# ZihanLiao/pytorch-kaldi-resnet

Measured on AMD Instinct MI355X. Metric: utterances/sec (300-frame x 80 fbank, bs256/GPU), ResNet-34 + AAM-softmax training step, higher is better.
Workload: dtype f32 (operands as 2 fp16 terms of value x 2^k, 3 cross products, f32 accumulate); 1 GPU; BASELINE configs[1]: ResNet-34 + AAM-softmax (m 0.2, s 30), 1211 speakers, 300-frame x 80 fbank, per-GPU batch 256, fwd+CE+bwd+SGD(0.9, wd 5e-4); global_batch=256, frames=300, feat_dim=80, parallelism=dp1, launch=hipGraph replay (1 graph), mfma=f16x3

## Files before the change

### include/spkhip.h

```cpp
#ifndef SPKHIP_H
#define SPKHIP_H
#include <stddef.h>
#ifdef __cplusplus
extern "C" {
#endif

int spk_version(void);
const char* spk_last_error(void);
int spk_build_flags(void);

#define SPK_IN_AFFINE_RELU 1
#define SPK_EPI_AFFINE 2
#define SPK_EPI_ADD 4
#define SPK_EPI_RELU 8
#define SPK_EPI_STATS 16
#define SPK_IN_BNBWD 64
#define SPK_EPI_BNBWD 32

#define SPK_CONV_WS 128
#define SPK_CONV_PIPE 1024

#define SPK_CONV_M16 (1 << 17)

#define SPK_WGRAD_GROUPS 2048
// ... 33 lines not shown
                      unsigned* side_amax, const int* wlen , void* stream);

int spk_conv_wgrad_limits(int WN, int* max_halo_pix , int* max_tile_pix );
size_t spk_conv_wgrad_workspace(int nsplit, int ksize, int Cin, int Cout);
int spk_conv3x3_c32_stream(const float* in, const float* wpk, float* out, const float* in_scale, const float* in_shift, float* stats,
                           int B, int H, int W, int flags, const unsigned* in_amax, unsigned* out_amax, int nblocks, void* stream);
int spk_conv1x1_stream(const float* in, const float* wpk, float* out, const float* in_scale, const float* in_shift,
                       const float* epi_add, const unsigned* add_mask, const float* bn_raw, const unsigned* bn_mask,
                       const float* bn4, float* stats, long long P, int C, int flags, const unsigned* in_amax, unsigned* out_amax,
                       int nblocks, void* stream);
int spk_conv1x1_stream_rows(int nblocks, int C);
int spk_wgrad_reduce(const float* partial, float* dw, int nslab, int ksize, int Cin, int Cout, int accumulate, void* stream);
int spk_conv_wgrad(const float* x, const float* dy, float* dw, float* partial, const float* in_scale,
                   const float* in_shift, int B, int IH, int IW, int Cin, int OH, int OW, int Cout, int ksize, int stride,
                   int TH, int TW, int WN, int nsplit, int flags, int accumulate, int split , const unsigned* dy_amax , const unsigned* x_amax , void* stream);

int spk_stem_fwd_blocks(int B, int F, int T);
int spk_stem_conv_fwd(const float* x, const float* w, float* out, float* stats, const float* epi_scale,
                      const float* epi_shift, int B, int F, int T, int flags,
                      unsigned* amax_out , void* stream);
int spk_stem_conv_fwd_len(const float* x, const float* w, float* out, float* stats, const float* epi_scale,
                          const float* epi_shift, int B, int F, int T, int flags, unsigned* amax_out, const int* len ,
                          void* stream);
int spk_stem_wgrad_blocks(int B, int F, int T);
int spk_stem_conv_wgrad(const float* x, const float* draw, float* dw, float* partial, int B, int F, int T,
                        int accumulate, void* stream);
int spk_stem_stats(const float* x, const float* w, float* stats, int B, int F, int T, void* stream);
int spk_stem_fwd_apply(const float* x, const float* w, const float* scale, const float* shift, float* raw_out, float* act_out,
                       unsigned* mask_out, unsigned* amax_out, int B, int F, int T, void* stream);
int spk_stem_bwd_wgrad(const float* x, const float* d, const float* raw, const float* mean, const float* invstd,
// ... 156 lines not shown
```

### pytorch-kaldi-resnet_amd/csrc/conv_kernel.h

```cpp
#pragma once
#include "spk_common.h"
#include <type_traits>

#ifndef STAGE_U
#define STAGE_U 4
#endif
#ifndef CONV_NT
#define CONV_NT 3
#endif
static __device__ __forceinline__ void conv_st(float* p, f32x4 v) {
    if constexpr ((CONV_NT & 1) != 0) __builtin_nontemporal_store(v, (f32x4*)p);
    else *(f32x4*)p = v;
}
template <int BIT>
static __device__ __forceinline__ f32x4 conv_ld(const float* p) {
    if constexpr ((CONV_NT & BIT) != 0) return __builtin_nontemporal_load((const f32x4*)p);
    else return *(const f32x4*)p;
}
#ifndef STAGE_U2
#define STAGE_U2 2
#endif
#ifndef STAGE_U2_C32
#define STAGE_U2_C32 4
#endif
// ... 42 lines not shown
    int halo_h, halo_w, min_dy, min_dx;
    unsigned halo_w_magic;
    int ntaps, ncg, nblocks, flags;
    int tap_off[18];
    int tap_w[18];
    int tap_g[18];
    const unsigned* in_amax;
    float in_sigma;
    const unsigned* w_amax;
    unsigned* out_amax;
    unsigned* side_amax;
    const int* wlen;
    int tap_boff[9];
    int kc;
};

#define PIPE_D 3
#ifndef PIPE16_D
#define PIPE16_D 3
#endif
#ifndef PIPE16_D_CONV
#define PIPE16_D_CONV 3
#endif
#ifndef PIPE_VPM
#define PIPE_VPM 6
#endif
#ifdef CONV_STAMPS
#define CONV_STAMP_BLOCKS 4096
static __device__ unsigned long long g_conv_stamps[CONV_STAMP_BLOCKS][16];
#define STAMP(i) do { if (threadIdx.x == 0 && blockIdx.x < CONV_STAMP_BLOCKS) g_conv_stamps[blockIdx.x][i] = __builtin_amdgcn_s_memtime(); } while (0)
// ... 1121 lines not shown
```

### pytorch-kaldi-resnet_amd/csrc/conv_mfma.hip

```cpp
#include "conv_kernel.h"

int spk_launch_conv_split(const ConvArgs& a, size_t lds_bytes, int MT, int NT, int split, int ck, hipStream_t st);
int spk_launch_conv_pipe(const ConvArgs& a, size_t lds_bytes, int MT, int NT, hipStream_t st);
int spk_launch_conv_ws(const ConvArgs& a, int MT, int NT, int WC, int split, int lp4, hipStream_t st);

template <int MT, int NT>
static int launch_conv(const ConvArgs& a, size_t lds_bytes, hipStream_t st) {
    if (a.flags & SPK_IN_BNBWD)
        hipLaunchKernelGGL((conv_mfma_kernel<MT, NT, true, 0>), dim3(a.nblocks), dim3(256), lds_bytes, st, a);
    else if (a.flags & SPK_EPI_WMASK)
        hipLaunchKernelGGL((conv_mfma_kernel<MT, NT, false, 0, SPK_EPI_WMASK>), dim3(a.nblocks), dim3(256), lds_bytes, st, a);
    else
        hipLaunchKernelGGL((conv_mfma_kernel<MT, NT, false, 0>), dim3(a.nblocks), dim3(256), lds_bytes, st, a);
    SPK_LAUNCH_CHECK("spk_conv_mfma");
    return 0;
}

static int conv_mfma_entry(const float* in, const float* wpk, float* out, const float* in_scale,
                             const float* in_shift, const float* epi_scale, const float* epi_shift,
                             const float* epi_add, const float* in_raw, const float* in_act, const float* in_bn4,
                             const float* in_coef, const unsigned* in_mask, const unsigned* bn_mask, const unsigned* add_mask, float* side_draw,
                             float* side_dz,
                             const float* bn_raw,
                             const float* bn_act, const float* bn4, float* stats, int B, int IH, int IW, int Cin, int OH,
// ... 137 lines not shown
            SPK_REQUIRE((Cin / SPK_SPLIT_CK) % 2 == 0, "spk_conv_mfma: CONV_M16 walks the 16-channel planes in pairs");
        }
        a.flags = flags & ~SPK_CONV_PIPE;
        return spk_launch_conv_pipe(a, lds2, MT, NT, st);
    }
    if (split) return spk_launch_conv_split(a, lds_bytes, MT, NT, split, ck, st);
#define CASE(M, N) if (MT == M && NT == N) return launch_conv<M, N>(a, lds_bytes, st)
    CASE(1, 1); CASE(2, 1); CASE(3, 1); CASE(4, 1);
    CASE(1, 2); CASE(2, 2); CASE(3, 2); CASE(4, 2);
    CASE(1, 4); CASE(2, 4);
#undef CASE
    spk_set_error("spk_conv_mfma: unsupported tile config MT=%d NT=%d", MT, NT);
    return -1;
}

extern "C" int spk_conv_mfma(const float* in, const float* wpk, float* out, const float* in_scale,
                             const float* in_shift, const float* epi_scale, const float* epi_shift,
                             const float* epi_add, const float* in_raw, const float* in_act, const float* in_bn4,
                             const float* in_coef, const unsigned* in_mask, const unsigned* bn_mask, const unsigned* add_mask, float* side_draw,
                             float* side_dz, const float* bn_raw, const float* bn_act, const float* bn4, float* stats, int B, int IH,
                             int IW, int Cin, int OH, int OW, int OHf, int OWf, int Cout, int IS, int OS, int ooy, int oox, int ntaps,
                             const int* tap_dy, const int* tap_dx, const int* tap_w, int TH, int TW, int MT,
                             int NT, int kc, int ips, int flags, int split, const unsigned* in_amax, unsigned* out_amax,
                             unsigned* side_amax, void* stream) {
    return conv_mfma_entry(in, wpk, out, in_scale, in_shift, epi_scale, epi_shift, epi_add, in_raw, in_act, in_bn4, in_coef, in_mask,
                           bn_mask, add_mask, side_draw, side_dz, bn_raw, bn_act, bn4, stats, B, IH, IW, Cin, OH, OW, OHf, OWf, Cout, IS,
                           OS, ooy, oox, ntaps, tap_dy, tap_dx, tap_w, TH, TW, MT, NT, kc, ips, flags, split, in_amax, out_amax,
                           side_amax, nullptr, stream);
}

// ... 16 lines not shown
```

### pytorch-kaldi-resnet_amd/csrc/conv_pipe.hip

```cpp
#include "conv_kernel.h"

template <int MT, int NT>
static int launch_pipe(const ConvArgs& a, size_t lds_bytes, hipStream_t st) {
    if (a.flags & SPK_IN_BNBWD) {
#ifndef SPK_EXPERIMENTAL
        spk_set_error("spk_conv_mfma: the pipelined fused-BatchNorm-backward kernel is an experimental form: build with SPK_EXPERIMENTAL=1");
        return -1;
#else
        if constexpr (MT * NT <= 4) {
            SPK_REQUIRE(a.in_mask, "spk_conv_mfma: the pipelined fused-BatchNorm-backward kernel takes the ReLU mask as sign bits");
            hipLaunchKernelGGL((conv_pipe_kernel<MT, NT, true, true>), dim3(a.nblocks), dim3(256), lds_bytes, st, a);
        } else {
            spk_set_error("spk_conv_mfma: no pipelined fused-BatchNorm-backward kernel for MT=%d NT=%d", MT, NT);
            return -1;
        }
#endif
    } else if (a.flags & SPK_CONV_M16) {
        ConvArgs b = a;
        b.flags = a.flags & ~SPK_CONV_M16;
        if constexpr (MT == 3 && NT == 2) {
            const int var = b.flags | (b.add_mask ? SPK_FL_ADDMASK : 0) | (b.bn_mask ? SPK_FL_BNMASK : 0) | (b.bn_act ? (1 << 30) : 0);
#define LP(PREV, VV) hipLaunchKernelGGL((conv_pipe_kernel<MT, NT, false, false, PREV, true, VV>), dim3(a.nblocks), dim3(256), lds_bytes, st, b)
            if (b.flags & SPK_EPI_WMASK) {
                LP(false, SPK_EPI_WMASK);
                SPK_LAUNCH_CHECK("spk_conv_mfma(pipe)");
                return 0;
            }
#ifdef SPK_NO_FL_VARIANTS
            if (a.flags & SPK_IN_PRESPLIT) LP(true, -1); else LP(false, -1);
#else
            switch (var) {
#ifdef SPK_FL_FWD_PIPE
                case SPK_IN_AFFINE_RELU | SPK_EPI_STATS: LP(false, SPK_IN_AFFINE_RELU | SPK_EPI_STATS); break;
                case SPK_EPI_STATS: LP(false, SPK_EPI_STATS); break;
#endif
                case SPK_IN_PRESPLIT | SPK_EPI_STATS | SPK_EPI_BNBWD: LP(true, SPK_IN_PRESPLIT | SPK_EPI_STATS | SPK_EPI_BNBWD); break;
                case SPK_IN_PRESPLIT | SPK_EPI_ADD | SPK_EPI_STATS | SPK_EPI_BNBWD | SPK_FL_ADDMASK | SPK_FL_BNMASK:
                    LP(true, SPK_IN_PRESPLIT | SPK_EPI_ADD | SPK_EPI_STATS | SPK_EPI_BNBWD | SPK_FL_ADDMASK | SPK_FL_BNMASK); break;
                case SPK_IN_PRESPLIT | SPK_EPI_ADD | SPK_FL_ADDMASK: LP(true, SPK_IN_PRESPLIT | SPK_EPI_ADD | SPK_FL_ADDMASK); break;
                default:
                    if (a.flags & SPK_IN_PRESPLIT) LP(true, -1); else LP(false, -1);
            }
#endif
#undef LP
        } else {
            spk_set_error("spk_conv_mfma: no 16x16x32 pipelined kernel for MT=%d NT=%d", MT, NT);
            return -1;
        }
    } else if (a.flags & SPK_EPI_WMASK)
        hipLaunchKernelGGL((conv_pipe_kernel<MT, NT, false, false, false, false, SPK_EPI_WMASK>), dim3(a.nblocks), dim3(256), lds_bytes, st, a);
    else if (a.flags & SPK_IN_PRESPLIT)
        hipLaunchKernelGGL((conv_pipe_kernel<MT, NT, false, false, true>), dim3(a.nblocks), dim3(256), lds_bytes, st, a);
    else
        hipLaunchKernelGGL((conv_pipe_kernel<MT, NT, false>), dim3(a.nblocks), dim3(256), lds_bytes, st, a);
    SPK_LAUNCH_CHECK("spk_conv_mfma(pipe)");
    return 0;
}

int spk_launch_conv_pipe(const ConvArgs& a, size_t lds_bytes, int MT, int NT, hipStream_t st) {
#define CASE(M, N) if (MT == M && NT == N) return launch_pipe<M, N>(a, lds_bytes, st);
    CASE(2, 1) CASE(3, 1) CASE(1, 2) CASE(2, 2) CASE(3, 2) CASE(1, 4)
#undef CASE
    spk_set_error("spk_conv_mfma: unsupported pipelined tile config MT=%d NT=%d", MT, NT);
    return -1;
}

#ifdef CONV_STAMPS
extern "C" int spk_debug_stamps_pipe(unsigned long long* out, int nblocks) {
    if (nblocks < 0) {
// ... 9 lines not shown
```

### pytorch-kaldi-resnet_amd/csrc/conv_split.hip

```cpp
#include "conv_kernel.h"

template <int MT, int NT>
static int launch_split_ck32(const ConvArgs& a, size_t lds_bytes, hipStream_t st) {
#ifndef SPK_NO_FL_VARIANTS
    const int var = a.flags | (a.add_mask ? SPK_FL_ADDMASK : 0) | (a.bn_mask ? SPK_FL_BNMASK : 0) | (a.in_mask ? SPK_FL_INMASK : 0);
    constexpr int V2 = SPK_IN_BNBWD | SPK_SIDE_PRESPLIT | SPK_EPI_STATS | SPK_EPI_BNBWD | SPK_FL_INMASK;
    constexpr int V1 = SPK_IN_BNBWD | SPK_SIDE_PRESPLIT | SPK_EPI_ADD | SPK_EPI_STATS | SPK_EPI_BNBWD | SPK_FL_ADDMASK | SPK_FL_BNMASK;
    if (!a.in_act && !a.bn_act && !a.side_dz && var == V2)
        hipLaunchKernelGGL((conv_mfma_kernel<MT, NT, true, 3, V2, 32>), dim3(a.nblocks), dim3(256), lds_bytes, st, a);
    else if (!a.in_act && !a.bn_act && !a.side_dz && var == V1)
        hipLaunchKernelGGL((conv_mfma_kernel<MT, NT, true, 3, V1, 32>), dim3(a.nblocks), dim3(256), lds_bytes, st, a);
    else
#endif
        hipLaunchKernelGGL((conv_mfma_kernel<MT, NT, true, 3, -1, 32>), dim3(a.nblocks), dim3(256), lds_bytes, st, a);
    SPK_LAUNCH_CHECK("spk_conv_mfma(split, 32-channel planes)");
    return 0;
}

template <int MT, int NT, int SPLIT>
static int launch_split(const ConvArgs& a, size_t lds_bytes, hipStream_t st) {
    if (a.flags & SPK_IN_BNBWD) {
#ifndef SPK_NO_FL_VARIANTS
        if constexpr (SPLIT == 3 && MT == 2 && NT == 1) {
            const int var = a.flags | (a.add_mask ? SPK_FL_ADDMASK : 0) | (a.bn_mask ? SPK_FL_BNMASK : 0) | (a.in_mask ? SPK_FL_INMASK : 0);
            constexpr int V2 = SPK_IN_BNBWD | SPK_SIDE_PRESPLIT | SPK_EPI_STATS | SPK_EPI_BNBWD | SPK_FL_INMASK;
            constexpr int V1 = SPK_IN_BNBWD | SPK_SIDE_PRESPLIT | SPK_EPI_ADD | SPK_EPI_STATS | SPK_EPI_BNBWD | SPK_FL_ADDMASK | SPK_FL_BNMASK;
            if (!a.in_act && !a.bn_act && !a.side_dz && (var == V1 || var == V2)) {
                if (var == V2) hipLaunchKernelGGL((conv_mfma_kernel<MT, NT, true, SPLIT, V2>), dim3(a.nblocks), dim3(256), lds_bytes, st, a);
                else hipLaunchKernelGGL((conv_mfma_kernel<MT, NT, true, SPLIT, V1>), dim3(a.nblocks), dim3(256), lds_bytes, st, a);
                SPK_LAUNCH_CHECK("spk_conv_mfma(split)");
                return 0;
            }
        }
#endif
        hipLaunchKernelGGL((conv_mfma_kernel<MT, NT, true, SPLIT>), dim3(a.nblocks), dim3(256), lds_bytes, st, a);
    } else if (a.flags & SPK_EPI_WMASK) {
        hipLaunchKernelGGL((conv_mfma_kernel<MT, NT, false, SPLIT, SPK_EPI_WMASK>), dim3(a.nblocks), dim3(256), lds_bytes, st, a);
    } else {
#ifndef SPK_NO_FL_VARIANTS
        if constexpr (SPLIT == 3 && ((MT == 2 && NT == 1) || (MT == 1 && NT == 2) || (MT == 2 && NT == 2))) {
            if (!a.add_mask && !a.bn_mask && !a.bn_act) {
                if (a.flags == (SPK_IN_AFFINE_RELU | SPK_EPI_STATS)) {
                    hipLaunchKernelGGL((conv_mfma_kernel<MT, NT, false, SPLIT, SPK_IN_AFFINE_RELU | SPK_EPI_STATS>), dim3(a.nblocks), dim3(256), lds_bytes, st, a);
                    SPK_LAUNCH_CHECK("spk_conv_mfma(split)");
                    return 0;
                }
                if (a.flags == SPK_EPI_STATS) {
                    hipLaunchKernelGGL((conv_mfma_kernel<MT, NT, false, SPLIT, SPK_EPI_STATS>), dim3(a.nblocks), dim3(256), lds_bytes, st, a);
                    SPK_LAUNCH_CHECK("spk_conv_mfma(split)");
                    return 0;
                }
            }
        }
#endif
        hipLaunchKernelGGL((conv_mfma_kernel<MT, NT, false, SPLIT>), dim3(a.nblocks), dim3(256), lds_bytes, st, a);
    }
    SPK_LAUNCH_CHECK("spk_conv_mfma(split)");
    return 0;
}

int spk_launch_conv_split(const ConvArgs& a, size_t lds_bytes, int MT, int NT, int split, int ck, hipStream_t st) {
    if (ck == 32) {
        if (MT == 2 && NT == 1) return launch_split_ck32<2, 1>(a, lds_bytes, st);
        if (MT == 1 && NT == 1) return launch_split_ck32<1, 1>(a, lds_bytes, st);
        spk_set_error("spk_conv_mfma: 32-channel planes are instantiated for MT=2 / MT=1 with NT=1, not MT=%d NT=%d", MT, NT);
        return -1;
    }
#define CASE(M, N)                                                      \
    if (MT == M && NT == N) {                                           \
// ... 22 lines not shown
```

### pytorch-kaldi-resnet_amd/csrc/conv_wgrad.hip

```cpp
#include "conv_wgrad.h"

int spk_launch_wgrad_split(const WgradArgs& a, int WN, int split, hipStream_t st);
int spk_launch_wgrad_ws(const WgradArgs& a, int WN, hipStream_t st);
int spk_launch_wgrad_pipe(const WgradArgs& a, int WN, hipStream_t st);
int spk_launch_wgrad_1x1(const WgradArgs& a, int WN, int CG, hipStream_t st);
int spk_launch_wgrad_wm16(const WgradArgs& a, hipStream_t st);
int spk_launch_wgrad_c32m16(const WgradArgs& a, hipStream_t st);
int spk_launch_wgrad_wm(const WgradArgs& a, hipStream_t st);

template <int NTAPS, int WK, int WN>
__global__ __launch_bounds__(256, 2) void conv_wgrad_kernel(WgradArgs a) {
    extern __shared__ __attribute__((aligned(16))) float lds[];
    const int tid = threadIdx.x, lane = tid & 63;
    const int wave = __builtin_amdgcn_readfirstlane(tid >> 6);
    const int r = lane & 31, h = lane >> 5;
    const int wk = wave / WN, wn = wave % WN;
    const int ci0 = blockIdx.y * 32;
    const int co0 = blockIdx.z * (32 * WN);
    const int halo_pix = a.halo_h * a.halo_w;
    const int npix = a.TH * a.TW;
    float* xs = lds;
    float* dys = lds + halo_pix * 32;
    const int flags = a.flags;

// ... 160 lines not shown
            }
        }
    }
    if (wk == 0) {
        float* slab = a.partial + (size_t)blockIdx.x * NTAPS * a.Cin * a.Cout;
#pragma unroll
        for (int t = 0; t < NTAPS; ++t)
#pragma unroll
            for (int e = 0; e < 16; ++e) {
                const int row = (e & 3) + 8 * (e >> 2) + 4 * h;
                slab[((size_t)t * a.Cin + ci0 + row) * a.Cout + co0 + wn * 32 + r] = acc[t][e];
            }
    }
}

__global__ void wgrad_reduce_kernel(const float* __restrict__ partial, float* __restrict__ dw, int nslab, int ntaps,
                                    int Cin, int Cout, int accumulate) {
    const int idx = blockIdx.x * blockDim.x + threadIdx.x;
    const int total = ntaps * Cin * Cout;
    if (idx >= total) return;
    float s0 = 0.f, s1 = 0.f, s2 = 0.f, s3 = 0.f;
    int k = 0;
    for (; k + 4 <= nslab; k += 4) {
        s0 += partial[(size_t)(k + 0) * total + idx];
        s1 += partial[(size_t)(k + 1) * total + idx];
        s2 += partial[(size_t)(k + 2) * total + idx];
        s3 += partial[(size_t)(k + 3) * total + idx];
    }
    for (; k < nslab; ++k) s0 += partial[(size_t)k * total + idx];
    const float s = (s0 + s1) + (s2 + s3);
    const int co = idx % Cout;
    const int ci = (idx / Cout) % Cin;
    const int t = idx / (Cout * Cin);
    float* dst = dw + ((size_t)co * Cin + ci) * ntaps + t;
    *dst = accumulate ? *dst + s : s;
}

// ... 12 lines not shown
    return 0;
}

extern "C" size_t spk_conv_wgrad_workspace(int nsplit, int ksize, int Cin, int Cout) {
    return (size_t)nsplit * ksize * ksize * Cin * Cout * sizeof(float);
}

extern "C" int spk_wgrad_reduce(const float* partial, float* dw, int nslab, int ksize, int Cin, int Cout, int accumulate,
                                void* stream) {
    SPK_REQUIRE(partial && dw && nslab >= 1 && (ksize == 1 || ksize == 3), "spk_wgrad_reduce: bad arguments");
    const int ntaps = ksize * ksize, total = ntaps * Cin * Cout;
    hipLaunchKernelGGL(wgrad_reduce_kernel, dim3(spk_ceil_div(total, 256)), dim3(256), 0, (hipStream_t)stream, partial, dw, nslab,
                       ntaps, Cin, Cout, accumulate);
    SPK_LAUNCH_CHECK("spk_wgrad_reduce");
    return 0;
}

extern "C" int spk_conv_wgrad(const float* x, const float* dy, float* dw, float* partial, const float* in_scale,
                              const float* in_shift, int B, int IH, int IW, int Cin, int OH, int OW, int Cout,
                              int ksize, int stride, int TH, int TW, int WN, int nsplit, int flags, int accumulate,
                              int split, const unsigned* dy_amax, const unsigned* x_amax, void* stream) {
    SPK_REQUIRE(x && dy && dw && partial, "spk_conv_wgrad: null pointer");
    SPK_REQUIRE(!(flags & SPK_EPI_WMASK), "spk_conv_wgrad: SPK_EPI_WMASK is a forward-epilogue flag (spk_conv_mfma_len)");
    SPK_REQUIRE(ksize == 1 || ksize == 3, "spk_conv_wgrad: ksize=%d unsupported", ksize);
    SPK_REQUIRE(Cin % 32 == 0 && Cout % 32 == 0, "spk_conv_wgrad: channels (%d,%d) must be multiples of 32", Cin, Cout);
    SPK_REQUIRE(WN == 1 || WN == 2 || WN == 4, "spk_conv_wgrad: WN=%d", WN);
    SPK_REQUIRE(Cout % (32 * WN) == 0, "spk_conv_wgrad: Cout=%d not a multiple of 32*WN", Cout);
    SPK_REQUIRE(TH >= 1 && TW >= 2 && (TW % 2) == 0, "spk_conv_wgrad: TW=%d must be even", TW);
    SPK_REQUIRE(nsplit >= 1, "spk_conv_wgrad: nsplit");
    SPK_REQUIRE(!(flags & SPK_IN_AFFINE_RELU) || (in_scale && in_shift), "spk_conv_wgrad: IN_AFFINE_RELU needs scale/shift");
// ... 80 lines not shown
```

### pytorch-kaldi-resnet_amd/csrc/conv_wgrad_split.hip

```cpp
#include "conv_wgrad.h"

typedef short s16x4 __attribute__((ext_vector_type(4)));
typedef short s16x8 __attribute__((ext_vector_type(8)));
typedef __attribute__((address_space(3))) s16x4 lds_s16x4;

static __device__ __forceinline__ s16x8 tr_read8(const unsigned char* p0, const unsigned char* p1) {
#ifdef WG_ABL_NO_FRAG
    s16x8 v = {1, 2, 3, 4, 5, 6, 7, 8};
    asm volatile("" : "+v"(v) : "v"(p0), "v"(p1));
    return v;
#endif
    const s16x4 lo = __builtin_amdgcn_ds_read_tr16_b64_v4i16((lds_s16x4*)p0);
    const s16x4 hi = __builtin_amdgcn_ds_read_tr16_b64_v4i16((lds_s16x4*)p1);
    return __builtin_shufflevector(lo, hi, 0, 1, 2, 3, 4, 5, 6, 7);
}

#ifndef WGRAD_XCD_BAND
#define WGRAD_XCD_BAND 1
#endif
struct WgradBlock { int g, ci0, co0; };
template <int WN>
static __device__ __forceinline__ WgradBlock wgrad_block(const WgradArgs& a) {
    const int ncgi = a.Cin >> 5, M = ncgi * (a.Cout / (32 * WN));
    const int bid = blockIdx.x;
// ... 493 lines not shown
    if (a.halo_h * a.halo_w <= 32 * 4) hipLaunchKernelGGL((conv_wgrad_ws_kernel<NTAPS, WK, WN, 4>), grid, dim3(512), lds_bytes, st, a);
    else hipLaunchKernelGGL((conv_wgrad_ws_kernel<NTAPS, WK, WN, WGRAD_NX>), grid, dim3(512), lds_bytes, st, a);
    SPK_LAUNCH_CHECK("spk_conv_wgrad(ws)");
    return 0;
}

int spk_launch_wgrad_ws(const WgradArgs& a, int WN, hipStream_t st) {
    SPK_REQUIRE(a.KW == 3, "spk_conv_wgrad(ws): 3x3 only");
    if (WN == 1) return launch_ws<9, 4, 1>(a, st);
    if (WN == 2) return launch_ws<9, 2, 2>(a, st);
    return launch_ws<9, 1, 4>(a, st);
}

#endif

template <int NTAPS, int WK, int WN>
static int launch_one(const WgradArgs& a, int split, hipStream_t st) {
    const int npix_pad = ((a.TH * a.TW + 15) >> 4) << 4;
    constexpr int PD = WN * 192 + (WN > 1 ? 64 : 0);
    size_t lds_bytes = (size_t)a.halo_h * a.halo_w * 192 + (size_t)npix_pad * PD;
    const size_t red_bytes = (WK > 1) ? (size_t)WN * NTAPS * 16 * 64 * sizeof(float) : 0;
    if (lds_bytes < red_bytes) lds_bytes = red_bytes;
    SPK_REQUIRE(lds_bytes <= 160 * 1024, "spk_conv_wgrad(split): tile %dx%d needs %zu B of LDS", a.TH, a.TW, lds_bytes);
    dim3 grid(a.nsplit * (a.Cin / 32) * (a.Cout / (32 * WN)));
    const bool small = a.halo_h * a.halo_w <= 32 * 4;
    if (split == 3) {
        const int var = ((a.flags & SPK_IN_AFFINE_RELU) ? 1 : 0) | ((a.flags & SPK_DY_PRESPLIT) ? 2 : 0);
        if constexpr (NTAPS == 9 && WK == 4 && WN == 1) {
            if (!small && var == 3) {
                hipLaunchKernelGGL((conv_wgrad_split_kernel<NTAPS, WK, WN, 3, WGRAD_NX, 3>), grid, dim3(256), lds_bytes, st, a);
                SPK_LAUNCH_CHECK("spk_conv_wgrad(split)");
                return 0;
            }
            if (!small && var == 2) {
                hipLaunchKernelGGL((conv_wgrad_split_kernel<NTAPS, WK, WN, 3, WGRAD_NX, 2>), grid, dim3(256), lds_bytes, st, a);
                SPK_LAUNCH_CHECK("spk_conv_wgrad(split)");
                return 0;
            }
        }
        if (small) hipLaunchKernelGGL((conv_wgrad_split_kernel<NTAPS, WK, WN, 3, 4>), grid, dim3(256), lds_bytes, st, a);
        else hipLaunchKernelGGL((conv_wgrad_split_kernel<NTAPS, WK, WN, 3, WGRAD_NX>), grid, dim3(256), lds_bytes, st, a);
    } else if constexpr (NTAPS == 9) {
        if (split == 6) {
            if (small) hipLaunchKernelGGL((conv_wgrad_split_kernel<9, WK, WN, 6, 4>), grid, dim3(256), lds_bytes, st, a);
            else hipLaunchKernelGGL((conv_wgrad_split_kernel<9, WK, WN, 6, WGRAD_NX>), grid, dim3(256), lds_bytes, st, a);
        } else {
            if (small) hipLaunchKernelGGL((conv_wgrad_split_kernel<9, WK, WN, 9, 4>), grid, dim3(256), lds_bytes, st, a);
            else hipLaunchKernelGGL((conv_wgrad_split_kernel<9, WK, WN, 9, WGRAD_NX>), grid, dim3(256), lds_bytes, st, a);
        }
    } else {
        spk_set_error("spk_conv_wgrad(split): 1x1 weight gradients exist in the f16x3 mode only");
        return -1;
    }
    SPK_LAUNCH_CHECK("spk_conv_wgrad(split)");
    return 0;
// ... 13 lines not shown
```

### pytorch-kaldi-resnet_amd/csrc/err.cpp

```cpp
#include <stdarg.h>
#include <stdio.h>
#include "spk_common.h"

static thread_local char g_err[512] = "";

void spk_set_error(const char* fmt, ...) {
    va_list ap;
    va_start(ap, fmt);
    vsnprintf(g_err, sizeof(g_err), fmt, ap);
    va_end(ap);
}

extern "C" const char* spk_last_error(void) { return g_err; }
extern "C" int spk_version(void) { return 300; }
extern "C" int spk_build_flags(void) {
#ifdef SPK_EXPERIMENTAL
    return 1;
#else
    return 0;
#endif
}
```

### pytorch-kaldi-resnet_amd/csrc/spk_common.h

```cpp
#pragma once
#include <hip/hip_runtime.h>
#include <stdint.h>

typedef float f32x4 __attribute__((ext_vector_type(4)));
typedef float f32x16 __attribute__((ext_vector_type(16)));

void spk_set_error(const char* fmt, ...);
#define SPK_REQUIRE(cond, ...)                 \
    do {                                       \
        if (!(cond)) {                         \
            spk_set_error(__VA_ARGS__);        \
            return -1;                         \
        }                                      \
    } while (0)
#define SPK_LAUNCH_CHECK(name)                                                          \
    do {                                                                                \
        hipError_t e__ = hipGetLastError();                                             \
        if (e__ != hipSuccess) {                                                        \
            spk_set_error("%s: launch failed: %s", name, hipGetErrorString(e__));       \
            return (int)e__;                                                            \
        }                                                                               \
    } while (0)

enum {
// ... 6 lines not shown
    SPK_IN_BNBWD = 64,
    SPK_CONV_WS = 128,
    SPK_CONV_PIPE = 1024,
    SPK_WGRAD_GROUPS = 2048,
    SPK_IN_PRESPLIT = 1 << 14,
    SPK_SIDE_PRESPLIT = 1 << 15,
    SPK_DY_PRESPLIT = 1 << 16,
    SPK_CONV_M16 = 1 << 17,
    SPK_WGRAD_NOSHIFT = 1 << 18,
    SPK_WGRAD_M16 = 1 << 19,
    SPK_CONV_CK32 = 1 << 23,
    SPK_EPI_WMASK = 1 << 24
};

static inline int spk_ceil_div(int a, int b) { return (a + b - 1) / b; }

typedef __bf16 bf16x8 __attribute__((ext_vector_type(8)));
#ifdef __HIPCC__
static __device__ __forceinline__ unsigned pack_bf16x2(float lo, float hi, float& rlo, float& rhi) {
    const __bf16 a = (__bf16)lo, b = (__bf16)hi;
    rlo = lo - (float)a;
    rhi = hi - (float)b;
    return (unsigned)__builtin_bit_cast(unsigned short, a) | ((unsigned)__builtin_bit_cast(unsigned short, b) << 16);
}
static __device__ __forceinline__ void split3(f32x4 w, uint2& t0, uint2& t1, uint2& t2) {
    float r0, r1, r2, r3, q0, q1, q2, q3;
    t0.x = pack_bf16x2(w[0], w[1], r0, r1);
    t0.y = pack_bf16x2(w[2], w[3], r2, r3);
    t1.x = pack_bf16x2(r0, r1, q0, q1);
    t1.y = pack_bf16x2(r2, r3, q2, q3);
// ... 59 lines not shown
```

### pytorch-kaldi-resnet_amd/hip.py

```python
import ctypes
import os

import torch

_HERE = os.path.dirname(os.path.abspath(__file__))
LIB_PATH = os.environ.get("SPK_LIB", os.path.join(_HERE, "libspkhip.so"))

IN_AFFINE_RELU, EPI_AFFINE, EPI_ADD, EPI_RELU, EPI_STATS, EPI_BNBWD, IN_BNBWD, CONV_WS = 1, 2, 4, 8, 16, 32, 64, 128
CONV_PIPE = 1024
WGRAD_GROUPS = 2048
IN_PRESPLIT, SIDE_PRESPLIT, DY_PRESPLIT = 1 << 14, 1 << 15, 1 << 16
CONV_M16 = 1 << 17
CONV_CK32 = 1 << 23
WGRAD_NOSHIFT = 1 << 18
WGRAD_M16 = 1 << 19
EPI_WMASK = 1 << 24
MASK_NONE, MASK_ACT, MASK_RAW, MASK_BITS = 0, 1, 2, 3

_P = ctypes.c_void_p
_I = ctypes.c_int
_L = ctypes.c_longlong
_F = ctypes.c_float
_D = ctypes.c_double
_IP = ctypes.POINTER(ctypes.c_int)

_SIGS = {
    "spk_pack_conv_weight": [_P, _P, _I, _I, _I, _I, _I, _P],
    "spk_pack_conv_weight_split": [_P, _P, _I, _I, _I, _I, _I, _I, _P],
    "spk_pack_job_bytes": [],
    "spk_build_flags": [],
    "spk_pack_conv_weights_batched": [_P, _I, _I, _I, _P],
    "spk_conv_mfma": [_P] * 21 + [_I] * 14 + [_IP, _IP, _IP] + [_I] * 8 + [_P, _P, _P, _P],
    "spk_conv_mfma_len": [_P] * 21 + [_I] * 14 + [_IP, _IP, _IP] + [_I] * 8 + [_P, _P, _P, _P, _P],
    "spk_conv3x3_c32_stream": [_P] * 6 + [_I] * 4 + [_P, _P, _I, _P],
    "spk_conv1x1_stream": [_P] * 11 + [_L, _I, _I, _P, _P, _I, _P],
    "spk_conv1x1_stream_rows": [_I, _I],
    "spk_conv_wgrad": [_P] * 6 + [_I] * 16 + [_P, _P, _P],
    "spk_conv_wgrad_limits": [_I, _IP, _IP],
    "spk_wgrad_reduce": [_P, _P, _I, _I, _I, _I, _I, _P],
    "spk_stem_fwd_blocks": [_I, _I, _I],
    "spk_stem_conv_fwd": [_P] * 6 + [_I] * 4 + [_P, _P],
    "spk_stem_conv_fwd_len": [_P] * 6 + [_I] * 4 + [_P, _P, _P],
    "spk_stem_wgrad_blocks": [_I, _I, _I],
    "spk_stem_conv_wgrad": [_P] * 4 + [_I] * 4 + [_P],
    "spk_stem_stats": [_P] * 3 + [_I] * 3 + [_P],
    "spk_stem_fwd_apply": [_P] * 8 + [_I] * 3 + [_P],
    "spk_stem_bwd_wgrad": [_P] * 10 + [_I] * 4 + [_P],
    "spk_bn_stats_blocks": [_L, _I],
    "spk_bn_stats_partial": [_P, _P, _L, _I, _P],
    "spk_bn_finalize": [_P, _I, _I, _D] + [_P] * 9 + [_F, _F, _P, _P, _P, _P],
    "spk_bn_eval_coeffs": [_P] * 6 + [_I, _F, _P],
    "spk_bn_apply": [_P] * 8 + [_L, _I, _I, _P, _P],
    "spk_bn_bwd_reduce": [_P] * 8 + [_L, _I, _I, _P, _P],
    "spk_bn_bwd_finalize": [_P, _I, _I, _D] + [_P] * 5 + [_I, _P, _P, _P, _P, _P, _P, _P],
# ... 136 lines not shown
```

Measured before the change: 5521 utt/s.

## Centralize flag-specialized kernel variant selection and widen variant coverage

New measurement: 5636 utt/s, median of 6. 2.1% higher.

```diff
diff --git a/include/spkhip.h b/include/spkhip.h
--- a/include/spkhip.h
+++ b/include/spkhip.h
@@ -71,6 +71,15 @@
 int spk_conv_wgrad(const float* x, const float* dy, float* dw, float* partial, const float* in_scale,
                    const float* in_shift, int B, int IH, int IW, int Cin, int OH, int OW, int Cout, int ksize, int stride,
                    int TH, int TW, int WN, int nsplit, int flags, int accumulate, int split , const unsigned* dy_amax , const unsigned* x_amax , void* stream);
+
+#define SPK_PTR_ADD_MASK 1
+#define SPK_PTR_BN_MASK 2
+#define SPK_PTR_IN_MASK 4
+#define SPK_PTR_IN_ACT 8
+#define SPK_PTR_BN_ACT 16
+#define SPK_PTR_SIDE_DZ 32
+int spk_conv_variant_of(int MT, int NT, int split, int flags, int ptrs);
+int spk_wgrad_variant_of(int ksize, int stride, int TH, int TW, int WN, int split, int flags);
 
 int spk_stem_fwd_blocks(int B, int F, int T);
 int spk_stem_conv_fwd(const float* x, const float* w, float* out, float* stats, const float* epi_scale,
diff --git a/pytorch-kaldi-resnet_amd/csrc/conv_kernel.h b/pytorch-kaldi-resnet_amd/csrc/conv_kernel.h
--- a/pytorch-kaldi-resnet_amd/csrc/conv_kernel.h
+++ b/pytorch-kaldi-resnet_amd/csrc/conv_kernel.h
@@ -80,6 +80,11 @@
     int tap_boff[9];
     int kc;
 };
+
+static inline int conv_ptr_pattern(const ConvArgs& a) {
+    return (a.add_mask ? SPK_PTR_ADD_MASK : 0) | (a.bn_mask ? SPK_PTR_BN_MASK : 0) | (a.in_mask ? SPK_PTR_IN_MASK : 0) |
+           (a.in_act ? SPK_PTR_IN_ACT : 0) | (a.bn_act ? SPK_PTR_BN_ACT : 0) | (a.side_dz ? SPK_PTR_SIDE_DZ : 0);
+}
 
 #define PIPE_D 3
 #ifndef PIPE16_D
diff --git a/pytorch-kaldi-resnet_amd/csrc/conv_mfma.hip b/pytorch-kaldi-resnet_amd/csrc/conv_mfma.hip
--- a/pytorch-kaldi-resnet_amd/csrc/conv_mfma.hip
+++ b/pytorch-kaldi-resnet_amd/csrc/conv_mfma.hip
@@ -175,6 +175,14 @@
     return -1;
 }
 
+extern "C" int spk_conv_variant_of(int MT, int NT, int split, int flags, int ptrs) {
+    if (flags & SPK_CONV_WS) return -1;
+    const int ck = (flags & SPK_CONV_CK32) ? 32 : SPK_SPLIT_CK;
+    flags &= ~SPK_CONV_CK32;
+    if (flags & SPK_CONV_PIPE) return split == 3 ? spk_pipe_variant_of(MT, NT, flags & ~SPK_CONV_PIPE, ptrs) : -1;
+    return split ? spk_split_variant_of(MT, NT, split, ck, flags, ptrs) : -1;
+}
+
 extern "C" int spk_conv_mfma(const float* in, const float* wpk, float* out, const float* in_scale,
                              const float* in_shift, const float* epi_scale, const float* epi_shift,
                              const float* epi_add, const float* in_raw, const float* in_act, const float* in_bn4,
diff --git a/pytorch-kaldi-resnet_amd/csrc/conv_pipe.hip b/pytorch-kaldi-resnet_amd/csrc/conv_pipe.hip
--- a/pytorch-kaldi-resnet_amd/csrc/conv_pipe.hip
+++ b/pytorch-kaldi-resnet_amd/csrc/conv_pipe.hip
@@ -1,7 +1,56 @@
 #include "conv_kernel.h"
+
+constexpr int FLP_DGRAD_BN = SPK_IN_PRESPLIT | SPK_EPI_STATS | SPK_EPI_BNBWD;
+constexpr int FLP_DGRAD_ADD_BN = SPK_IN_PRESPLIT | SPK_EPI_ADD | SPK_EPI_STATS | SPK_EPI_BNBWD | SPK_FL_ADDMASK | SPK_FL_BNMASK;
+constexpr int FLP_DGRAD_ADD = SPK_IN_PRESPLIT | SPK_EPI_ADD | SPK_FL_ADDMASK;
+constexpr int FLP_FWD_AFF = SPK_IN_AFFINE_RELU | SPK_EPI_STATS;
+constexpr int FLP_FWD = SPK_EPI_STATS;
+
+static constexpr bool pipe_has_fl(int MT, int NT, bool m16, int fl) {
+    if (!m16 || !(MT == 3 && NT == 2)) return false;
+#ifdef SPK_FL_FWD_PIPE
+    if (fl == FLP_FWD_AFF || fl == FLP_FWD) return true;
+#endif
+    return fl == FLP_DGRAD_BN || fl == FLP_DGRAD_ADD_BN || fl == FLP_DGRAD_ADD;
+}
+
+int spk_pipe_variant_of(int MT, int NT, int flags, int ptrs) {
+#ifdef SPK_NO_FL_VARIANTS
+    return -1;
+#else
+    if (!spk_fl_variants_enabled() || (flags & (SPK_EPI_WMASK | SPK_IN_BNBWD)) || (ptrs & SPK_PTR_BN_ACT)) return -1;
+    const bool m16 = (flags & SPK_CONV_M16) != 0;
+    const int fl = (flags & ~SPK_CONV_M16) | ((ptrs & SPK_PTR_ADD_MASK) ? SPK_FL_ADDMASK : 0) | ((ptrs & SPK_PTR_BN_MASK) ? SPK_FL_BNMASK : 0);
+    return pipe_has_fl(MT, NT, m16, fl) ? fl : -1;
+#endif
+}
+
+template <int MT, int NT>
+static bool launch_pipe_fl(int fl, const ConvArgs& b, size_t lds_bytes, hipStream_t st) {
+#ifndef SPK_NO_FL_VARIANTS
+#define FL_CASE(V)                                                                                                         \
+    case V:                                                                                                                \
+        if constexpr (pipe_has_fl(MT, NT, true, V)) {                                                                      \
+            hipLaunchKernelGGL((conv_pipe_kernel<MT, NT, false, false, ((V) & SPK_IN_PRESPLIT) != 0, true, V>), dim3(b.nblocks), \
+                               dim3(256), lds_bytes, st, b);                                                               \
+            return true;                                                                                                   \
+        }                                                                                                                  \
+        break;
+    switch (fl) {
+        FL_CASE(FLP_FWD_AFF)
+        FL_CASE(FLP_FWD)
+        FL_CASE(FLP_DGRAD_BN)
+        FL_CASE(FLP_DGRAD_ADD_BN)
+        FL_CASE(FLP_DGRAD_ADD)
+    }
+#undef FL_CASE
+#endif
+    return false;
+}
 
 template <int MT, int NT>
 static int launch_pipe(const ConvArgs& a, size_t lds_bytes, hipStream_t st) {
+    const int fl = spk_pipe_variant_of(MT, NT, a.flags, conv_ptr_pattern(a));
     if (a.flags & SPK_IN_BNBWD) {
 #ifndef SPK_EXPERIMENTAL
         spk_set_error("spk_conv_mfma: the pipelined fused-BatchNorm-backward kernel is an experimental form: build with SPK_EXPERIMENTAL=1");
@@ -19,40 +68,31 @@
         ConvArgs b = a;
         b.flags = a.flags & ~SPK_CONV_M16;
         if constexpr (MT == 3 && NT == 2) {
-            const int var = b.flags | (b.add_mask ? SPK_FL_ADDMASK : 0) | (b.bn_mask ? SPK_FL_BNMASK : 0) | (b.bn_act ? (1 << 30) : 0);
 #define LP(PREV, VV) hipLaunchKernelGGL((conv_pipe_kernel<MT, NT, false, false, PREV, true, VV>), dim3(a.nblocks), dim3(256), lds_bytes, st, b)
             if (b.flags & SPK_EPI_WMASK) {
                 LP(false, SPK_EPI_WMASK);
-                SPK_LAUNCH_CHECK("spk_conv_mfma(pipe)");
-                return 0;
+            } else if (fl >= 0) {
+                if (!launch_pipe_fl<MT, NT>(fl, b, lds_bytes, st)) {
+                    spk_set_error("spk_conv_mfma: no instance of flag variant 0x%x of the 16x16x32 pipelined kernel", fl);
+                    return -1;
+                }
+            } else if (a.flags & SPK_IN_PRESPLIT) {
+                LP(true, -1);
+            } else {
+                LP(false, -1);
             }
-#ifdef SPK_NO_FL_VARIANTS
-            if (a.flags & SPK_IN_PRESPLIT) LP(true, -1); else LP(false, -1);
-#else
-            switch (var) {
-#ifdef SPK_FL_FWD_PIPE
-                case SPK_IN_AFFINE_RELU | SPK_EPI_STATS: LP(false, SPK_IN_AFFINE_RELU | SPK_EPI_STATS); break;
-                case SPK_EPI_STATS: LP(false, SPK_EPI_STATS); break;
-#endif
-                case SPK_IN_PRESPLIT | SPK_EPI_STATS | SPK_EPI_BNBWD: LP(true, SPK_IN_PRESPLIT | SPK_EPI_STATS | SPK_EPI_BNBWD); break;
-                case SPK_IN_PRESPLIT | SPK_EPI_ADD | SPK_EPI_STATS | SPK_EPI_BNBWD | SPK_FL_ADDMASK | SPK_FL_BNMASK:
-                    LP(true, SPK_IN_PRESPLIT | SPK_EPI_ADD | SPK_EPI_STATS | SPK_EPI_BNBWD | SPK_FL_ADDMASK | SPK_FL_BNMASK); break;
-                case SPK_IN_PRESPLIT | SPK_EPI_ADD | SPK_FL_ADDMASK: LP(true, SPK_IN_PRESPLIT | SPK_EPI_ADD | SPK_FL_ADDMASK); break;
-                default:
-                    if (a.flags & SPK_IN_PRESPLIT) LP(true, -1); else LP(false, -1);
-            }
-#endif
 #undef LP
         } else {
             spk_set_error("spk_conv_mfma: no 16x16x32 pipelined kernel for MT=%d NT=%d", MT, NT);
             return -1;
         }
-    } else if (a.flags & SPK_EPI_WMASK)
+    } else if (a.flags & SPK_EPI_WMASK) {
         hipLaunchKernelGGL((conv_pipe_kernel<MT, NT, false, false, false, false, SPK_EPI_WMASK>), dim3(a.nblocks), dim3(256), lds_bytes, st, a);
-    else if (a.flags & SPK_IN_PRESPLIT)
+    } else if (a.flags & SPK_IN_PRESPLIT) {
         hipLaunchKernelGGL((conv_pipe_kernel<MT, NT, false, false, true>), dim3(a.nblocks), dim3(256), lds_bytes, st, a);
-    else
+    } else {
         hipLaunchKernelGGL((conv_pipe_kernel<MT, NT, false>), dim3(a.nblocks), dim3(256), lds_bytes, st, a);
+    }
     SPK_LAUNCH_CHECK("spk_conv_mfma(pipe)");
     return 0;
 }
diff --git a/pytorch-kaldi-resnet_amd/csrc/conv_split.hip b/pytorch-kaldi-resnet_amd/csrc/conv_split.hip
--- a/pytorch-kaldi-resnet_amd/csrc/conv_split.hip
+++ b/pytorch-kaldi-resnet_amd/csrc/conv_split.hip
@@ -1,58 +1,102 @@
 #include "conv_kernel.h"
+
+constexpr int FLV_BNBWD2 = SPK_IN_BNBWD | SPK_SIDE_PRESPLIT | SPK_EPI_STATS | SPK_EPI_BNBWD | SPK_FL_INMASK;
+constexpr int FLV_BNBWD1 = SPK_IN_BNBWD | SPK_SIDE_PRESPLIT | SPK_EPI_ADD | SPK_EPI_STATS | SPK_EPI_BNBWD | SPK_FL_ADDMASK | SPK_FL_BNMASK;
+constexpr int FLV_FWD_AFF = SPK_IN_AFFINE_RELU | SPK_EPI_STATS;
+constexpr int FLV_FWD = SPK_EPI_STATS;
+constexpr int FLV_DGRAD_PAIR = SPK_IN_PRESPLIT;
+constexpr int FLV_DGRAD_ADD = SPK_EPI_ADD;
+
+static constexpr bool split_has_fl(int MT, int NT, int ck, int fl) {
+    const bool t21 = MT == 2 && NT == 1, t12 = MT == 1 && NT == 2, t22 = MT == 2 && NT == 2, t32 = MT == 3 && NT == 2;
+    if (ck == 32) return (t21 || (MT == 1 && NT == 1)) && (fl == FLV_BNBWD1 || fl == FLV_BNBWD2);
+    switch (fl) {
+        case FLV_BNBWD1: case FLV_BNBWD2: return t21;
+        case FLV_FWD_AFF: return t21 || t12 || t22;
+        case FLV_FWD: return t21 || t12 || t22 || t32 || (MT == 1 && NT == 4);
+        case FLV_DGRAD_PAIR: case FLV_DGRAD_ADD: return t21 || t22 || t32;
+    }
+    return false;
+}
+
+int spk_split_variant_of(int MT, int NT, int split, int ck, int flags, int ptrs) {
+#ifdef SPK_NO_FL_VARIANTS
+    return -1;
+#else
+    if (!spk_fl_variants_enabled() || split != 3 || (flags & SPK_EPI_WMASK)) return -1;
+    int fl = flags;
+    if (flags & SPK_IN_BNBWD) {
+        if (ptrs & (SPK_PTR_IN_ACT | SPK_PTR_BN_ACT | SPK_PTR_SIDE_DZ)) return -1;
+        fl |= ((ptrs & SPK_PTR_ADD_MASK) ? SPK_FL_ADDMASK : 0) | ((ptrs & SPK_PTR_BN_MASK) ? SPK_FL_BNMASK : 0) |
+              ((ptrs & SPK_PTR_IN_MASK) ? SPK_FL_INMASK : 0);
+    } else if (ptrs & (SPK_PTR_ADD_MASK | SPK_PTR_BN_MASK | SPK_PTR_BN_ACT)) {
+        return -1;
+    }
+    return split_has_fl(MT, NT, ck, fl) ? fl : -1;
+#endif
+}
+
+#define FL_CASE(V, CK)                                                                                                                \
+    case V:                                                                                                                           \
+        if constexpr (split_has_fl(MT, NT, CK, V)) {                                                                                  \
+            hipLaunchKernelGGL((conv_mfma_kernel<MT, NT, ((V) & SPK_IN_BNBWD) != 0, 3, V, CK>), dim3(a.nblocks), dim3(256), lds_bytes, st, a); \
+            return true;                                                                                                              \
+        }                                                                                                                             \
+        break;
+
+template <int MT, int NT>
+static bool launch_fl_ck32(int fl, const ConvArgs& a, size_t lds_bytes, hipStream_t st) {
+#ifndef SPK_NO_FL_VARIANTS
+    switch (fl) {
+        FL_CASE(FLV_BNBWD2, 32)
+        FL_CASE(FLV_BNBWD1, 32)
+    }
+#endif
+    return false;
+}
 
 template <int MT, int NT>
 static int launch_split_ck32(const ConvArgs& a, size_t lds_bytes, hipStream_t st) {
-#ifndef SPK_NO_FL_VARIANTS
-    const int var = a.flags | (a.add_mask ? SPK_FL_ADDMASK : 0) | (a.bn_mask ? SPK_FL_BNMASK : 0) | (a.in_mask ? SPK_FL_INMASK : 0);
-    constexpr int V2 = SPK_IN_BNBWD | SPK_SIDE_PRESPLIT | SPK_EPI_STATS | SPK_EPI_BNBWD | SPK_FL_INMASK;
-    constexpr int V1 = SPK_IN_BNBWD | SPK_SIDE_PRESPLIT | SPK_EPI_ADD | SPK_EPI_STATS | SPK_EPI_BNBWD | SPK_FL_ADDMASK | SPK_FL_BNMASK;
-    if (!a.in_act && !a.bn_act && !a.side_dz && var == V2)
-        hipLaunchKernelGGL((conv_mfma_kernel<MT, NT, true, 3, V2, 32>), dim3(a.nblocks), dim3(256), lds_bytes, st, a);
-    else if (!a.in_act && !a.bn_act && !a.side_dz && var == V1)
-        hipLaunchKernelGGL((conv_mfma_kernel<MT, NT, true, 3, V1, 32>), dim3(a.nblocks), dim3(256), lds_bytes, st, a);
-    else
-#endif
+    const int fl = spk_split_variant_of(MT, NT, 3, 32, a.flags, conv_ptr_pattern(a));
+    if (fl < 0)
         hipLaunchKernelGGL((conv_mfma_kernel<MT, NT, true, 3, -1, 32>), dim3(a.nblocks), dim3(256), lds_bytes, st, a);
+    else if (!launch_fl_ck32<MT, NT>(fl, a, lds_bytes, st)) {
+        spk_set_error("spk_conv_mfma: no instance of flag variant 0x%x for MT=%d NT=%d (32-channel planes)", fl, MT, NT);
+        return -1;
+    }
     SPK_LAUNCH_CHECK("spk_conv_mfma(split, 32-channel planes)");
     return 0;
 }
 
+template <int MT, int NT>
+static bool launch_fl(int fl, const ConvArgs& a, size_t lds_bytes, hipStream_t st) {
+#ifndef SPK_NO_FL_VARIANTS
+    switch (fl) {
+        FL_CASE(FLV_BNBWD2, SPK_SPLIT_CK)
+        FL_CASE(FLV_BNBWD1, SPK_SPLIT_CK)
+        FL_CASE(FLV_FWD_AFF, SPK_SPLIT_CK)
+        FL_CASE(FLV_FWD, SPK_SPLIT_CK)
+        FL_CASE(FLV_DGRAD_PAIR, SPK_SPLIT_CK)
+        FL_CASE(FLV_DGRAD_ADD, SPK_SPLIT_CK)
+    }
+#endif
+    return false;
+}
+#undef FL_CASE
+
 template <int MT, int NT, int SPLIT>
 static int launch_split(const ConvArgs& a, size_t lds_bytes, hipStream_t st) {
-    if (a.flags & SPK_IN_BNBWD) {
-#ifndef SPK_NO_FL_VARIANTS
-        if constexpr (SPLIT == 3 && MT == 2 && NT == 1) {
-            const int var = a.flags | (a.add_mask ? SPK_FL_ADDMASK : 0) | (a.bn_mask ? SPK_FL_BNMASK : 0) | (a.in_mask ? SPK_FL_INMASK : 0);
-            constexpr int V2 = SPK_IN_BNBWD | SPK_SIDE_PRESPLIT | SPK_EPI_STATS | SPK_EPI_BNBWD | SPK_FL_INMASK;
-            constexpr int V1 = SPK_IN_BNBWD | SPK_SIDE_PRESPLIT | SPK_EPI_ADD | SPK_EPI_STATS | SPK_EPI_BNBWD | SPK_FL_ADDMASK | SPK_FL_BNMASK;
-            if (!a.in_act && !a.bn_act && !a.side_dz && (var == V1 || var == V2)) {
-                if (var == V2) hipLaunchKernelGGL((conv_mfma_kernel<MT, NT, true, SPLIT, V2>), dim3(a.nblocks), dim3(256), lds_bytes, st, a);
-                else hipLaunchKernelGGL((conv_mfma_kernel<MT, NT, true, SPLIT, V1>), dim3(a.nblocks), dim3(256), lds_bytes, st, a);
-                SPK_LAUNCH_CHECK("spk_conv_mfma(split)");
-                return 0;
-            }
+    const int fl = spk_split_variant_of(MT, NT, SPLIT, SPK_SPLIT_CK, a.flags, conv_ptr_pattern(a));
+    if (fl >= 0) {
+        if (!launch_fl<MT, NT>(fl, a, lds_bytes, st)) {
+            spk_set_error("spk_conv_mfma: no instance of flag variant 0x%x for MT=%d NT=%d", fl, MT, NT);
+            return -1;
         }
-#endif
+    } else if (a.flags & SPK_IN_BNBWD) {
         hipLaunchKernelGGL((conv_mfma_kernel<MT, NT, true, SPLIT>), dim3(a.nblocks), dim3(256), lds_bytes, st, a);
     } else if (a.flags & SPK_EPI_WMASK) {
         hipLaunchKernelGGL((conv_mfma_kernel<MT, NT, false, SPLIT, SPK_EPI_WMASK>), dim3(a.nblocks), dim3(256), lds_bytes, st, a);
     } else {
-#ifndef SPK_NO_FL_VARIANTS
-        if constexpr (SPLIT == 3 && ((MT == 2 && NT == 1) || (MT == 1 && NT == 2) || (MT == 2 && NT == 2))) {
-            if (!a.add_mask && !a.bn_mask && !a.bn_act) {
-                if (a.flags == (SPK_IN_AFFINE_RELU | SPK_EPI_STATS)) {
-                    hipLaunchKernelGGL((conv_mfma_kernel<MT, NT, false, SPLIT, SPK_IN_AFFINE_RELU | SPK_EPI_STATS>), dim3(a.nblocks), dim3(256), lds_bytes, st, a);
-                    SPK_LAUNCH_CHECK("spk_conv_mfma(split)");
-                    return 0;
-                }
-                if (a.flags == SPK_EPI_STATS) {
-                    hipLaunchKernelGGL((conv_mfma_kernel<MT, NT, false, SPLIT, SPK_EPI_STATS>), dim3(a.nblocks), dim3(256), lds_bytes, st, a);
-                    SPK_LAUNCH_CHECK("spk_conv_mfma(split)");
-                    return 0;
-                }
-            }
-        }
-#endif
         hipLaunchKernelGGL((conv_mfma_kernel<MT, NT, false, SPLIT>), dim3(a.nblocks), dim3(256), lds_bytes, st, a);
     }
     SPK_LAUNCH_CHECK("spk_conv_mfma(split)");
diff --git a/pytorch-kaldi-resnet_amd/csrc/conv_wgrad.hip b/pytorch-kaldi-resnet_amd/csrc/conv_wgrad.hip
--- a/pytorch-kaldi-resnet_amd/csrc/conv_wgrad.hip
+++ b/pytorch-kaldi-resnet_amd/csrc/conv_wgrad.hip
@@ -198,13 +198,31 @@
     }
 }
 
+#ifndef WGRAD_REDUCE_NF
+#define WGRAD_REDUCE_NF 16
+#endif
 __global__ void wgrad_reduce_kernel(const float* __restrict__ partial, float* __restrict__ dw, int nslab, int ntaps,
                                     int Cin, int Cout, int accumulate) {
+    static_assert(WGRAD_REDUCE_NF % 4 == 0, "the four chains take k = j (mod 4)");
     const int idx = blockIdx.x * blockDim.x + threadIdx.x;
     const int total = ntaps * Cin * Cout;
     if (idx >= total) return;
     float s0 = 0.f, s1 = 0.f, s2 = 0.f, s3 = 0.f;
     int k = 0;
+    if constexpr (WGRAD_REDUCE_NF > 4) {
+        for (; k + WGRAD_REDUCE_NF <= nslab; k += WGRAD_REDUCE_NF) {
+            float v[WGRAD_REDUCE_NF];
+#pragma unroll
+            for (int u = 0; u < WGRAD_REDUCE_NF; ++u) v[u] = partial[(size_t)(k + u) * total + idx];
+#pragma unroll
+            for (int u = 0; u < WGRAD_REDUCE_NF; u += 4) {
+                s0 += v[u + 0];
+                s1 += v[u + 1];
+                s2 += v[u + 2];
+                s3 += v[u + 3];
+            }
+        }
+    }
     for (; k + 4 <= nslab; k += 4) {
         s0 += partial[(size_t)(k + 0) * total + idx];
         s1 += partial[(size_t)(k + 1) * total + idx];
@@ -247,6 +265,11 @@
                        ntaps, Cin, Cout, accumulate);
     SPK_LAUNCH_CHECK("spk_wgrad_reduce");
     return 0;
+}
+
+extern "C" int spk_wgrad_variant_of(int ksize, int stride, int TH, int TW, int WN, int split, int flags) {
+    if (flags & (SPK_WGRAD_GROUPS | SPK_WGRAD_M16 | SPK_CONV_PIPE | SPK_CONV_WS)) return -1;
+    return spk_wgrad_split_variant_of(ksize, WN, split, flags, ((TH - 1) * stride + ksize) * ((TW - 1) * stride + ksize));
 }
 
 extern "C" int spk_conv_wgrad(const float* x, const float* dy, float* dw, float* partial, const float* in_scale,
diff --git a/pytorch-kaldi-resnet_amd/csrc/conv_wgrad_split.hip b/pytorch-kaldi-resnet_amd/csrc/conv_wgrad_split.hip
--- a/pytorch-kaldi-resnet_amd/csrc/conv_wgrad_split.hip
+++ b/pytorch-kaldi-resnet_amd/csrc/conv_wgrad_split.hip
@@ -531,6 +531,43 @@
 
 #endif
 
+static constexpr bool wgrad_split_has_var(int ntaps, int WN, bool small, int var) {
+    if (ntaps == 9 && WN == 1 && !small) return var == 2 || var == 3;
+    if (ntaps == 9 && WN == 2 && !small) return var == 2;
+    if (ntaps == 1 && WN == 2 && small) return var == 0;
+    return false;
+}
+
+int spk_wgrad_split_variant_of(int ksize, int WN, int split, int flags, int halo_pix) {
+#ifdef SPK_NO_FL_VARIANTS
+    return -1;
+#else
+    if (!spk_fl_variants_enabled() || split != 3) return -1;
+    const int var = ((flags & SPK_IN_AFFINE_RELU) ? 1 : 0) | ((flags & SPK_DY_PRESPLIT) ? 2 : 0);
+    return wgrad_split_has_var(ksize * ksize, WN, halo_pix <= 32 * 4, var) ? var : -1;
+#endif
+}
+
+template <int NTAPS, int WK, int WN, bool SMALL>
+static bool launch_var(int var, const WgradArgs& a, dim3 grid, size_t lds_bytes, hipStream_t st) {
+#ifndef SPK_NO_FL_VARIANTS
+#define VAR_CASE(V)                                                                                                              \
+    case V:                                                                                                                      \
+        if constexpr (wgrad_split_has_var(NTAPS, WN, SMALL, V)) {                                                                \
+            hipLaunchKernelGGL((conv_wgrad_split_kernel<NTAPS, WK, WN, 3, SMALL ? 4 : WGRAD_NX, V>), grid, dim3(256), lds_bytes, st, a); \
+            return true;                                                                                                         \
+        }                                                                                                                        \
+        break;
+    switch (var) {
+        VAR_CASE(0)
+        VAR_CASE(2)
+        VAR_CASE(3)
+    }
+#undef VAR_CASE
+#endif
+    return false;
+}
+
 template <int NTAPS, int WK, int WN>
 static int launch_one(const WgradArgs& a, int split, hipStream_t st) {
     const int npix_pad = ((a.TH * a.TW + 15) >> 4) << 4;
@@ -542,20 +579,13 @@
     dim3 grid(a.nsplit * (a.Cin / 32) * (a.Cout / (32 * WN)));
     const bool small = a.halo_h * a.halo_w <= 32 * 4;
     if (split == 3) {
-        const int var = ((a.flags & SPK_IN_AFFINE_RELU) ? 1 : 0) | ((a.flags & SPK_DY_PRESPLIT) ? 2 : 0);
-        if constexpr (NTAPS == 9 && WK == 4 && WN == 1) {
-            if (!small && var == 3) {
-                hipLaunchKernelGGL((conv_wgrad_split_kernel<NTAPS, WK, WN, 3, WGRAD_NX, 3>), grid, dim3(256), lds_bytes, st, a);
-                SPK_LAUNCH_CHECK("spk_conv_wgrad(split)");
-                return 0;
-            }
-            if (!small && var == 2) {
-                hipLaunchKernelGGL((conv_wgrad_split_kernel<NTAPS, WK, WN, 3, WGRAD_NX, 2>), grid, dim3(256), lds_bytes, st, a);
-                SPK_LAUNCH_CHECK("spk_conv_wgrad(split)");
-                return 0;
-            }
-        }
-        if (small) hipLaunchKernelGGL((conv_wgrad_split_kernel<NTAPS, WK, WN, 3, 4>), grid, dim3(256), lds_bytes, st, a);
+        const int var = spk_wgrad_split_variant_of(a.KW, WN, split, a.flags, a.halo_h * a.halo_w);
+        if (var >= 0) {
+            if (!(small ? launch_var<NTAPS, WK, WN, true>(var, a, grid, lds_bytes, st) : launch_var<NTAPS, WK, WN, false>(var, a, grid, lds_bytes, st))) {
+                spk_set_error("spk_conv_wgrad(split): no instance of variant %d for %d taps, WN=%d", var, NTAPS, WN);
+                return -1;
+            }
+        } else if (small) hipLaunchKernelGGL((conv_wgrad_split_kernel<NTAPS, WK, WN, 3, 4>), grid, dim3(256), lds_bytes, st, a);
         else hipLaunchKernelGGL((conv_wgrad_split_kernel<NTAPS, WK, WN, 3, WGRAD_NX>), grid, dim3(256), lds_bytes, st, a);
     } else if constexpr (NTAPS == 9) {
         if (split == 6) {
diff --git a/pytorch-kaldi-resnet_amd/csrc/err.cpp b/pytorch-kaldi-resnet_amd/csrc/err.cpp
--- a/pytorch-kaldi-resnet_amd/csrc/err.cpp
+++ b/pytorch-kaldi-resnet_amd/csrc/err.cpp
@@ -1,5 +1,6 @@
 #include <stdarg.h>
 #include <stdio.h>
+#include <stdlib.h>
 #include "spk_common.h"
 
 static thread_local char g_err[512] = "";
@@ -13,6 +14,14 @@
 
 extern "C" const char* spk_last_error(void) { return g_err; }
 extern "C" int spk_version(void) { return 300; }
+
+bool spk_fl_variants_enabled() {
+    static const bool on = [] {
+        const char* e = getenv("SPK_FL_VARIANTS");
+        return !(e && e[0] == '0' && e[1] == 0);
+    }();
+    return on;
+}
 extern "C" int spk_build_flags(void) {
 #ifdef SPK_EXPERIMENTAL
     return 1;
diff --git a/pytorch-kaldi-resnet_amd/csrc/spk_common.h b/pytorch-kaldi-resnet_amd/csrc/spk_common.h
--- a/pytorch-kaldi-resnet_amd/csrc/spk_common.h
+++ b/pytorch-kaldi-resnet_amd/csrc/spk_common.h
@@ -44,6 +44,19 @@
 };
 
 static inline int spk_ceil_div(int a, int b) { return (a + b - 1) / b; }
+
+enum {
+    SPK_PTR_ADD_MASK = 1,
+    SPK_PTR_BN_MASK = 2,
+    SPK_PTR_IN_MASK = 4,
+    SPK_PTR_IN_ACT = 8,
+    SPK_PTR_BN_ACT = 16,
+    SPK_PTR_SIDE_DZ = 32
+};
+bool spk_fl_variants_enabled();
+int spk_split_variant_of(int MT, int NT, int split, int ck, int flags, int ptrs);
+int spk_pipe_variant_of(int MT, int NT, int flags, int ptrs);
+int spk_wgrad_split_variant_of(int ksize, int WN, int split, int flags, int halo_pix);
 
 typedef __bf16 bf16x8 __attribute__((ext_vector_type(8)));
 #ifdef __HIPCC__
diff --git a/pytorch-kaldi-resnet_amd/hip.py b/pytorch-kaldi-resnet_amd/hip.py
--- a/pytorch-kaldi-resnet_amd/hip.py
+++ b/pytorch-kaldi-resnet_amd/hip.py
@@ -15,6 +15,7 @@
 WGRAD_NOSHIFT = 1 << 18
 WGRAD_M16 = 1 << 19
 EPI_WMASK = 1 << 24
+PTR_ADD_MASK, PTR_BN_MASK, PTR_IN_MASK, PTR_IN_ACT, PTR_BN_ACT, PTR_SIDE_DZ = 1, 2, 4, 8, 16, 32
 MASK_NONE, MASK_ACT, MASK_RAW, MASK_BITS = 0, 1, 2, 3
 
 _P = ctypes.c_void_p
@@ -38,6 +39,8 @@
     "spk_conv_wgrad": [_P] * 6 + [_I] * 16 + [_P, _P, _P],
     "spk_conv_wgrad_limits": [_I, _IP, _IP],
     "spk_wgrad_reduce": [_P, _P, _I, _I, _I, _I, _I, _P],
+    "spk_conv_variant_of": [_I, _I, _I, _I, _I],
+    "spk_wgrad_variant_of": [_I, _I, _I, _I, _I, _I, _I],
     "spk_stem_fwd_blocks": [_I, _I, _I],
     "spk_stem_conv_fwd": [_P] * 6 + [_I] * 4 + [_P, _P],
     "spk_stem_conv_fwd_len": [_P] * 6 + [_I] * 4 + [_P, _P, _P],
```
